# udaysankar01/xfeatSLAM

Hardware: AMD Instinct MI355X
Metric: XFeat frames/s (VGA, 4096 kpts) + 4096x4096 desc-match pairs/s (higher is better)
Workload: dtype f32

## Files before the change

### xfeatslam_amd/csrc/kernels_conv.hip

```cpp
#include "ctx.h"
#include "heads_kp4.hip.h"
#include <stdlib.h>

struct ConvArgs {
    const float* in;
    StatSrc st;
    size_t in_stride;
    int Hin, Win;
    const float* w;
    const float* bias;
    float* out;
    size_t out_stride;
    int Hout, Wout;
    double* part;
    size_t part_stride;
    int tiles_x;
    const float* pool; size_t pool_stride; const float* skip_w; const float* skip_b;
    const float* r4; size_t s4; int H4, W4; StatSrc st4;
    const float* r5; size_t s5; int H5, W5; StatSrc st5;
    const float* xstat; const float* w0; const float* bias0;
    int dbg;
};

enum { PRO_PLAIN = 0, PRO_BN = 1, PRO_IN = 2, PRO_B2IN = 3, PRO_FUSE = 4, PRO_L0 = 5, PRO_UNFOLD = 6, PRO_FUSEA = 7  };
enum { EPI_STATS = 0, EPI_BIAS = 1, EPI_BIAS_RELU = 2 };

#ifdef XFH_STAMPS
__device__ unsigned long long g_stamps[32 * 8];
#define XFH_STAMP(a, ph) do { if (blockIdx.x == gridDim.x / 2 && blockIdx.y == 0 && blockIdx.z == 0 && threadIdx.x == 0) g_stamps[((a).dbg & 31) * 8 + (ph)] = wall_clock64(); } while (0)
extern "C" int xfh_debug_stamps(unsigned long long* out) { return (int)hipMemcpyFromSymbol(out, HIP_SYMBOL(g_stamps), sizeof g_stamps); }
#define XFH_STAMP_ROW(row, ph) do { if (blockIdx.x == gridDim.x / 2 && blockIdx.y == 0 && blockIdx.z == 0 && threadIdx.x == 0) g_stamps[(row) * 8 + (ph)] = wall_clock64(); } while (0)
#else
#define XFH_STAMP(a, ph) do { } while (0)
#define XFH_STAMP_ROW(row, ph) do { } while (0)
#endif

__device__ __forceinline__ void lin_coeff_c(int in, int out, int d, int& i0, int& i1, float& l0, float& l1) {
    const float scale = (float)in / (float)out;
    float src = fmaf(scale, (float)d + 0.5f, -0.5f);
    if (src < 0.f) src = 0.f;
    int a = (int)src;
    if (a > in - 1) a = in - 1;
    float lam = src - (float)a;
    lam = fminf(fmaxf(lam, 0.f), 1.f);
    i0 = a; i1 = a + ((a < in - 1) ? 1 : 0);
    l1 = lam; l0 = 1.f - lam;
}
template <bool ACT = false>
__device__ __forceinline__ void ld_act8(const float* __restrict__ raw, const float* st, size_t pix, int g, f32x4& v0, f32x4& v1) {
    const float* p = raw + pix * 64 + g * 8;
    v0 = *(const f32x4*)p; v1 = *(const f32x4*)(p + 4);
    if constexpr (ACT) return;
#pragma unroll
    for (int q = 0; q < 4; ++q) {
        v0[q] = fmaxf(fmaf(v0[q], st[64 + g * 8 + q], st[g * 8 + q]), 0.f);
        v1[q] = fmaxf(fmaf(v1[q], st[64 + g * 8 + 4 + q], st[g * 8 + 4 + q]), 0.f);
    }
}
template <bool ACT = false>
__device__ __forceinline__ void up_bilinear8(const float* __restrict__ raw, const float* st, int Hi, int Wi, int Ho, int Wo, int y, int x, int g, f32x4& o0, f32x4& o1) {
    int y0, y1, x0, x1; float hy0, hy1, wx0, wx1;
    lin_coeff_c(Hi, Ho, y, y0, y1, hy0, hy1);
    lin_coeff_c(Wi, Wo, x, x0, x1, wx0, wx1);
    f32x4 a0, a1, b0, b1, c0, c1, d0, d1;
    ld_act8<ACT>(raw, st, (size_t)y0 * Wi + x0, g, a0, a1); ld_act8<ACT>(raw, st, (size_t)y0 * Wi + x1, g, b0, b1);
    ld_act8<ACT>(raw, st, (size_t)y1 * Wi + x0, g, c0, c1); ld_act8<ACT>(raw, st, (size_t)y1 * Wi + x1, g, d0, d1);
#pragma unroll
    for (int j = 0; j < 4; ++j) {
        const float t0 = fmaf(wx0, a0[j], wx1 * b0[j]), u0 = fmaf(wx0, c0[j], wx1 * d0[j]);
        o0[j] = fmaf(hy0, t0, hy1 * u0);
        const float t1 = fmaf(wx0, a1[j], wx1 * b1[j]), u1 = fmaf(wx0, c1[j], wx1 * d1[j]);
        o1[j] = fmaf(hy0, t1, hy1 * u1);
    }
}

__global__ __launch_bounds__(256)
void k_act_pyramid(const float* __restrict__ raw4, size_t s4, const float* __restrict__ st4, int n4 ,
                   const float* __restrict__ raw5, size_t s5, const float* __restrict__ st5, int n5, float* __restrict__ act4, float* __restrict__ act5) {
    const int b = blockIdx.z;
    for (int q = blockIdx.x * 256 + threadIdx.x; q < (n4 + n5) / 4; q += gridDim.x * 256) {
        const bool five = q >= n4 / 4;
        const int e = (five ? q - n4 / 4 : q) * 4, ch = e & 63;
        const float* st = (five ? st5 : st4) + (size_t)b * 128;
        const size_t off = (size_t)b * (five ? s5 : s4) + e;
        f32x4 v = *(const f32x4*)((five ? raw5 : raw4) + off);
        const f32x4 be = *(const f32x4*)(st + ch), al = *(const f32x4*)(st + 64 + ch);
#pragma unroll
        for (int j = 0; j < 4; ++j) v[j] = fmaxf(fmaf(v[j], al[j], be[j]), 0.f);
        *(f32x4*)((five ? act5 : act4) + off) = v;
    }
}

__global__ __launch_bounds__(256)
void k_bn_finalize(const double* __restrict__ part, size_t part_stride, int npart, int C, double count,
                   float* __restrict__ stat ) {
    __shared__ double red[256 * 2];
    const int b = blockIdx.x;
    bn_fold<16>(part + (size_t)b * part_stride, npart, C, count, stat + (size_t)b * 2 * C, red, threadIdx.x, 256);
}

__device__ __forceinline__ double wave_sum_f64(double v) {
    v += __shfl_xor(v, 32); v += __shfl_xor(v, 16); v += __shfl_xor(v, 8);
    v += __shfl_xor(v, 4); v += __shfl_xor(v, 2); v += __shfl_xor(v, 1);
    return v;
}
typedef float f32x2 __attribute__((ext_vector_type(2)));
__device__ __forceinline__ void l0_conv(const float (&win)[9], const XFH_CONST float* __restrict__ w, float (&acc)[4]) {
    f32x2 a0 = {0.f, 0.f}, a1 = {0.f, 0.f};
#pragma unroll
    for (int k = 0; k < 9; ++k) {
        const f32x2 v = {win[k], win[k]};
        a0 = __builtin_elementwise_fma(v, f32x2{w[k * 4], w[k * 4 + 1]}, a0);
        a1 = __builtin_elementwise_fma(v, f32x2{w[k * 4 + 2], w[k * 4 + 3]}, a1);
    }
    acc[0] = a0.x; acc[1] = a0.y; acc[2] = a1.x; acc[3] = a1.y;
}

constexpr int L0S_TW = 128, L0S_TH = 32, L0S_R = 4;
__global__ __launch_bounds__(256)
void k_block1_stats(const float* __restrict__ X, size_t x_stride, StatSrc xs, int H, int W, int tiles_x,
                    const float* __restrict__ w0, double* __restrict__ part, size_t part_stride, float* __restrict__ pool, size_t pool_stride) {
    __shared__ double s_red[512];
    __shared__ float s_xst[2];
    const int t = threadIdx.x, b = blockIdx.z, tile = blockIdx.x;
    XFH_STAMP_ROW(0, 0);
    const int gx = (tile % tiles_x) * L0S_TW + (t & 31) * 4, gy0 = (tile / tiles_x) * L0S_TH + (t >> 5) * L0S_R;
    const float* x = X + (size_t)b * x_stride;
    f32x4 rv[L0S_R + 2]; float rl[L0S_R + 2], rr[L0S_R + 2];
    {
        const int cx = min(gx, W - 4), cl = max(min(gx, W) - 1, 0), cr = min(gx + 4, W - 1);
#pragma unroll
        for (int i = 0; i < L0S_R + 2; ++i) {
            const float* p = x + (size_t)min(max(gy0 - 1 + i, 0), H - 1) * W;
            rv[i] = *(const f32x4*)(p + cx); rl[i] = p[cl]; rr[i] = p[cr];
        }
    }
    XFH_STAMP_ROW(0, 1);
    stage_stat<16>(xs, b, 1, tile == 0, s_xst, s_red, t, 256);
    XFH_STAMP_ROW(0, 2);
    const float m = s_xst[0], r = s_xst[1];
    auto load_row = [&](int i, float (&row)[6]) {
        const int gy = gy0 - 1 + i;
        const bool iny = gy >= 0 && gy < H;
        const f32x4 v = rv[i];
        const bool inx = iny && gx < W;
        row[1] = inx ? fmaf(v.x, r, m) : 0.f; row[2] = inx ? fmaf(v.y, r, m) : 0.f; row[3] = inx ? fmaf(v.z, r, m) : 0.f; row[4] = inx ? fmaf(v.w, r, m) : 0.f;
        row[0] = (iny && gx > 0 && gx - 1 < W) ? fmaf(rl[i], r, m) : 0.f;
        row[5] = (iny && gx + 4 < W) ? fmaf(rr[i], r, m) : 0.f;
    };
    float win[3][6];
    load_row(0, win[0]);
    load_row(1, win[1]);
    double sum[4] = {0.0, 0.0, 0.0, 0.0}, sq[4] = {0.0, 0.0, 0.0, 0.0};
    float ps = 0.f;
#pragma unroll
    for (int i = 0; i < L0S_R; ++i) {
        load_row(i + 2, win[(i + 2) % 3]);
        const float (&r0)[6] = win[i % 3], (&r1)[6] = win[(i + 1) % 3], (&r2)[6] = win[(i + 2) % 3];
#pragma unroll
        for (int q = 0; q < 4; ++q) ps += r1[q + 1];
#pragma unroll
        for (int q = 0; q < 4; ++q) {
            const float wq[9] = {r0[q], r0[q + 1], r0[q + 2], r1[q], r1[q + 1], r1[q + 2], r2[q], r2[q + 1], r2[q + 2]};
            float acc[4];
            l0_conv(wq, (const XFH_CONST float*)w0, acc);
            if (gy0 + i < H && gx + q < W) {
#pragma unroll
                for (int co = 0; co < 4; ++co) { const double d = (double)acc[co]; sum[co] += d; sq[co] = fma(d, d, sq[co]); }
            }
        }
    }
    XFH_STAMP_ROW(0, 4);
#pragma unroll
    for (int co = 0; co < 4; ++co) { sum[co] = wave_sum_f64(sum[co]); sq[co] = wave_sum_f64(sq[co]); }
    if (gy0 < H && gx < W) pool[(size_t)b * pool_stride + (size_t)(gy0 >> 2) * (W >> 2) + (gx >> 2)] = ps / 16.0f;
    if ((t & 63) == 0) {
#pragma unroll
        for (int co = 0; co < 4; ++co) { s_red[(t >> 6) * 8 + co * 2] = sum[co]; s_red[(t >> 6) * 8 + co * 2 + 1] = sq[co]; }
    }
    __syncthreads();
    if (t < 8)
        part[(size_t)b * part_stride + (size_t)tile * 8 + t] = (s_red[t] + s_red[8 + t]) + (s_red[16 + t] + s_red[24 + t]);
    XFH_STAMP_ROW(0, 5);
}

__device__ __forceinline__ int xcd_tile(int x, int n) {
    const int k = x & 7, q = n >> 3, r = n & 7;
    return k * q + (k < r ? k : r) + (x >> 3);
}

template <int CIN, int COUT, int ST, int PRO, bool FOLD, int EPI>
__global__ __launch_bounds__(256)
void k_conv_direct(ConvArgs a) {
    constexpr int TI = 15 * ST + 3;
    constexpr int SL = 256 / COUT;
    static_assert(PRO != PRO_L0 || (CIN == 4 && ST == 2 && COUT == 8), "PRO_L0 is block1.1");
    constexpr int XW = TI + 2, XS = XW + 1;
    constexpr int SIN = TI * TI * CIN > 256 * (COUT + 1) ? TI * TI * CIN : 256 * (COUT + 1);
    __shared__ __attribute__((aligned(16))) float s_in[SIN];
    float* s_out = s_in;
    __shared__ __attribute__((aligned(16))) float s_xwin[PRO == PRO_L0 ? XW * XS : 1];
    __shared__ double s_red[FOLD ? 512 : 8 * COUT];
    constexpr bool WLDS = FOLD;
    constexpr int NWQ = 9 * CIN * COUT / 4;
    __shared__ __attribute__((aligned(16))) float s_wt[WLDS ? NWQ * 4 : 4];
    const int t = threadIdx.x, b = blockIdx.z;
    XFH_STAMP(a, 0);
    const int tile = xcd_tile(blockIdx.x, gridDim.x), tx0 = (tile % a.tiles_x) * 16, ty0 = (tile / a.tiles_x) * 16;
    const float* in = a.in + (size_t)b * a.in_stride;
    __shared__ float s_stat[FOLD ? 2 * CIN : 1];
    static_assert(NWQ <= 256, "one weight quad per thread");
    f32x4 wq4 = {0.f, 0.f, 0.f, 0.f};
    if (WLDS && t < NWQ) wq4 = *(const f32x4*)(a.w + t * 4);
    const float* st = a.st.stat + (size_t)b * 2 * (PRO == PRO_IN ? 1 : CIN);

    constexpr int VEC = (CIN >= 4) ? 4 : 1;
    constexpr int G = CIN / VEC;
    if constexpr (PRO == PRO_L0) {
        float* s_x = s_xwin;
        const float xm = a.xstat[b * 2], xr = a.xstat[b * 2 + 1];
        constexpr int NX = (XW * XW + 255) / 256;
        float xv[NX];
#pragma unroll
        for (int k = 0; k < NX; ++k) {
            const int item = t + k * 256, iy = item / XW, ix = item % XW;
            const int gy = ty0 * ST - 2 + iy, gx = tx0 * ST - 2 + ix;
            xv[k] = in[(size_t)min(max(gy, 0), a.Hin - 1) * a.Win + min(max(gx, 0), a.Win - 1)];
        }
        if constexpr (FOLD) stage_stat<16>(a.st, b, CIN, tile == 0, s_stat, s_red, t, 256);
#pragma unroll
        for (int k = 0; k < NX; ++k) {
            const int item = t + k * 256, iy = item / XW, ix = item % XW;
            const int gy = ty0 * ST - 2 + iy, gx = tx0 * ST - 2 + ix;
            const bool ok = gy >= 0 && gy < a.Hin && gx >= 0 && gx < a.Win;
            if (item < XW * XW) s_x[iy * XS + ix] = ok ? fmaf(xv[k], xr, xm) : 0.f;
        }
        __syncthreads();
        for (int pix = t; pix < TI * TI; pix += 256) {
            const int iy = pix / TI, ix = pix % TI;
            const int gy = ty0 * ST - 1 + iy, gx = tx0 * ST - 1 + ix;
            f32x4 v = {0.f, 0.f, 0.f, 0.f};
            if (gy >= 0 && gy < a.Hin && gx >= 0 && gx < a.Win) {
                const float* sp = s_x + iy * XS + ix;
                const float win[9] = {sp[0], sp[1], sp[2], sp[XS], sp[XS + 1], sp[XS + 2], sp[2 * XS], sp[2 * XS + 1], sp[2 * XS + 2]};
                float acc[4];
                l0_conv(win, (const XFH_CONST float*)a.w0, acc);
#pragma unroll
                for (int q = 0; q < 4; ++q) {
                    if constexpr (EPI == EPI_BIAS_RELU) v[q] = fmaxf(acc[q] + a.bias0[q], 0.f);
                    else {
                        const float m = FOLD ? s_stat[q] : st[q], r = FOLD ? s_stat[CIN + q] : st[CIN + q];
                        v[q] = fmaxf(fmaf(acc[q], r, m), 0.f);
                    }
                }
            }
            *(f32x4*)(s_in + pix * CIN) = v;
        }
    } else
    {
        constexpr int NI = (TI * TI + 255) / 256;
        f32x4 iv[NI][G];
#pragma unroll
        for (int k = 0; k < NI; ++k) {
            const int pix = t + k * 256;
            const int gy = min(max(ty0 * ST - 1 + pix / TI, 0), a.Hin - 1), gx = min(max(tx0 * ST - 1 + pix % TI, 0), a.Win - 1);
            const float* p = in + ((size_t)gy * a.Win + gx) * CIN;
#pragma unroll
            for (int g = 0; g < G; ++g) {
                if constexpr (VEC == 4) iv[k][g] = *(const f32x4*)(p + g * 4);
                else iv[k][g].x = p[0];
            }
        }
        if constexpr (FOLD) stage_stat<16>(a.st, b, CIN, tile == 0, s_stat, s_red, t, 256);
#pragma unroll
        for (int k = 0; k < NI; ++k) {
            const int pix = t + k * 256;
            const int gy = ty0 * ST - 1 + pix / TI, gx = tx0 * ST - 1 + pix % TI;
            const bool ok = gy >= 0 && gy < a.Hin && gx >= 0 && gx < a.Win;
            if (pix >= TI * TI) continue;
            if constexpr (VEC == 4) {
#pragma unroll
                for (int g = 0; g < G; ++g) {
                    f32x4 v = iv[k][g];
#pragma unroll
                    for (int q = 0; q < 4; ++q) {
                        const float m = FOLD ? s_stat[g * 4 + q] : st[g * 4 + q], r = FOLD ? s_stat[CIN + g * 4 + q] : st[CIN + g * 4 + q];
                        v[q] = ok ? fmaxf(fmaf(v[q], r, m), 0.f) : 0.f;
                    }
                    *(f32x4*)(s_in + pix * CIN + g * 4) = v;
                }
            } else {
                s_in[pix] = ok ? fmaf(iv[k][0].x, st[1], st[0]) : 0.f;
            }
        }
    }
    if (WLDS && t < NWQ) *(f32x4*)(s_wt + t * 4) = wq4;
    __syncthreads();
    XFH_STAMP(a, 3);

    const int tx = t & 15, ty = t >> 4;
    float acc[COUT];
#pragma unroll
    for (int co = 0; co < COUT; ++co) acc[co] = 0.f;
#pragma unroll
    for (int ky = 0; ky < 3; ++ky)
#pragma unroll
        for (int kx = 0; kx < 3; ++kx) {
            const float* sp = s_in + ((ty * ST + ky) * TI + tx * ST + kx) * CIN;
            float v[CIN];
            if constexpr (VEC == 4) {
#pragma unroll
                for (int g = 0; g < G; ++g) {
                    const f32x4 q = *(const f32x4*)(sp + g * 4);
                    v[g * 4 + 0] = q.x; v[g * 4 + 1] = q.y; v[g * 4 + 2] = q.z; v[g * 4 + 3] = q.w;
                }
            } else {
                v[0] = sp[0];
            }
#pragma unroll
            for (int ci = 0; ci < CIN; ++ci) {
                if constexpr (WLDS) {
                    const float* wr = s_wt + ((ky * 3 + kx) * CIN + ci) * COUT;
#pragma unroll
                    for (int g4 = 0; g4 < COUT / 4; ++g4) {
                        const f32x4 w4 = *(const f32x4*)(wr + g4 * 4);
#pragma unroll
                        for (int e = 0; e < 4; ++e) acc[g4 * 4 + e] = fmaf(v[ci], w4[e], acc[g4 * 4 + e]);
                    }
                } else {
                    const float* wr = a.w + ((ky * 3 + kx) * CIN + ci) * COUT;
#pragma unroll
                    for (int co = 0; co < COUT; ++co) acc[co] = fmaf(v[ci], wr[co], acc[co]);
                }
            }
        }

    XFH_STAMP(a, 4);
    const int oy = ty0 + ty, ox = tx0 + tx;
    const bool valid = oy < a.Hout && ox < a.Wout;
    if constexpr (EPI == EPI_BIAS_RELU) {
#pragma unroll
        for (int co = 0; co < COUT; ++co) acc[co] = fmaxf(acc[co] + a.bias[co], 0.f);
    }
    if (valid) {
        float* o = a.out + (size_t)b * a.out_stride + ((size_t)oy * a.Wout + ox) * COUT;
#pragma unroll
        for (int g = 0; g < COUT / 4; ++g)
            *(f32x4*)(o + g * 4) = f32x4{acc[g * 4], acc[g * 4 + 1], acc[g * 4 + 2], acc[g * 4 + 3]};
    }
    if constexpr (EPI != EPI_STATS) return;
    __syncthreads();
#pragma unroll
    for (int co = 0; co < COUT; ++co) s_out[t * (COUT + 1) + co] = valid ? acc[co] : 0.f;
    __syncthreads();
    {
        const int c = t % COUT, j = t / COUT;
        double s = 0.0, ss = 0.0;
#pragma unroll
        for (int p = 0; p < 256 / SL; ++p) {
            const double v = (double)s_out[(j + p * SL) * (COUT + 1) + c];
            s += v; ss = fma(v, v, ss);
        }
#pragma unroll
        for (int off = COUT; off < 64; off <<= 1) { s += __shfl_xor(s, off); ss += __shfl_xor(ss, off); }
        if ((t & 63) < COUT) { s_red[((t >> 6) * COUT + c) * 2] = s; s_red[((t >> 6) * COUT + c) * 2 + 1] = ss; }
    }
    __syncthreads();
    if (t < 2 * COUT)
        a.part[(size_t)b * a.part_stride + (size_t)tile * COUT * 2 + t] = (s_red[t] + s_red[2 * COUT + t]) + (s_red[4 * COUT + t] + s_red[6 * COUT + t]);
    XFH_STAMP(a, 5);
}

typedef unsigned u32x4_t __attribute__((ext_vector_type(4)));
__device__ __forceinline__ __amdgpu_buffer_rsrc_t wbuf_make(const float* w) { return __builtin_amdgcn_make_buffer_rsrc((void*)w, 0, 0x7fffffff, 0x00020000); }
__device__ __forceinline__ f32x4 wbuf_ld(__amdgpu_buffer_rsrc_t r, int f , int chunk_float_off ) {
    return __builtin_bit_cast(f32x4, __builtin_amdgcn_raw_buffer_load_b128(r, (unsigned)f * 16u, chunk_float_off * 4, 0));
}
template <int COUT, int NT, int EPI>
__device__ __forceinline__ void conv_bias(const float* __restrict__ bias, int co0, float (&bv)[NT]) {
#pragma unroll
    for (int n = 0; n < NT; ++n) {
        bv[n] = 0.f;
        if constexpr (EPI != EPI_STATS) bv[n] = (COUT % 32 == 0 || co0 + n * 32 < COUT) ? bias[co0 + n * 32] : 0.f;
    }
}

template <int COUT, int NT, int WW, int WH, int EPI>
__device__ __forceinline__ void conv_epilogue(const f32x16 (&acc)[NT], float* __restrict__ wave_out , int Wout,
                                              int rows_left, int cols_left, int co0, int h, const float (&bias)[NT] ,
                                              double (&sum)[NT], double (&sq)[NT]) {
    static_assert(WW >= 8 && WW * WH == 32, "pixel block of a wave");
    XFH_MFMA_SETTLE();
    const bool full = rows_left >= WH && cols_left >= WW;
    const int lane_off = 4 * h * COUT + co0;
    const int rowstride = Wout * COUT;
    auto value = [&](int n, int r, float* dst, float bv) {
        float v = acc[n][r];
        if constexpr (EPI != EPI_STATS) v += bv;
        if constexpr (EPI == EPI_BIAS_RELU) v = fmaxf(v, 0.f);
        dst[lane_off] = v;
        if constexpr (EPI == EPI_STATS) { const double dv = (double)v; sum[n] += dv; sq[n] = fma(dv, dv, sq[n]); }
    };
    if (full) {
#pragma unroll
        for (int n = 0; n < NT; ++n) {
            sum[n] = 0.0; sq[n] = 0.0;
            if (COUT % 32 == 0 || co0 + n * 32 < COUT) {
#pragma unroll
                for (int r = 0; r < 16; ++r) {
                    const int pb = (r & 3) + 8 * (r >> 2);
                    value(n, r, wave_out + (pb / WW) * rowstride + (pb % WW) * COUT + n * 32, bias[n]);
                }
            }
        }
        return;
    }
#pragma unroll
    for (int n = 0; n < NT; ++n) {
        const int co = co0 + n * 32;
        sum[n] = 0.0; sq[n] = 0.0;
        const float bv = bias[n];
        const bool cok = COUT % 32 == 0 || co < COUT;
#pragma unroll
        for (int r = 0; r < 16; ++r) {
            const int pb = (r & 3) + 8 * (r >> 2);
            const int prow = pb / WW, pcol = pb % WW;
            float* dst = wave_out + prow * rowstride + pcol * COUT + n * 32;
            if (cok && prow < rows_left && pcol + 4 * h < cols_left) value(n, r, dst, bv);
        }
    }
}

#ifndef XFH_PD
#define XFH_PD 3
#endif

template <int CIN, int COUT, int KS, int ST, int WM, int WN, int NT, int WW, int PRO, int EPI, int CBMAX = 64, int TPC = 1, int PD = XFH_PD>
__device__ __forceinline__ void conv_mfma_body(const ConvArgs a, const int tile, const int b, float* smem) {
    constexpr int NTHR = 64 * WM * WN;
    constexpr int WH = 32 / WW, TH = WM * WH, TW = WW;
    constexpr int COUTP = WN * NT * 32;
    constexpr int PAD = KS / 2;
    constexpr int TIH = (TH - 1) * ST + KS, TIW = (TW - 1) * ST + KS;
    constexpr int CP = CIN + 4;
    constexpr int CB = CIN > CBMAX ? CBMAX : CIN;
    constexpr int NCB = CIN / CB;
    static_assert(TPC == 1 || NCB == 1, "several taps per chunk only with all channels in the chunk");
    static_assert((KS * KS) % TPC == 0, "taps per chunk");
    constexpr int NCHUNK = KS * KS * NCB / TPC;
    constexpr int NWBUF = NCHUNK > 1 ? 2 : 1;
    constexpr int KC = TPC * CB;
    constexpr int WS = KC + 4;
    constexpr int WCH = COUTP * KC;
    constexpr int NWLD = (WCH / 4 + NTHR - 1) / NTHR;
    constexpr int G = CIN / 8;
    constexpr int IN_FLOATS = TIH * TIW * CP;
    constexpr int W_FLOATS = COUTP * WS;

    float* s_in = smem;
    float* s_w = smem + IN_FLOATS;
    float* s_stat = s_w + NWBUF * W_FLOATS;

    const int t = threadIdx.x;
    const int tx0 = (tile % a.tiles_x) * TW, ty0 = (tile / a.tiles_x) * TH;
    const float* in = a.in + (size_t)b * a.in_stride;

    XFH_STAMP(a, 0);
    f32x4 wreg[PD][NWLD];
    const __amdgpu_buffer_rsrc_t wrs = wbuf_make(a.w);
#pragma unroll
    for (int c = 0; c < PD; ++c)
#pragma unroll
        for (int q = 0; q < NWLD; ++q) {
            const int f = t + q * NTHR;
            if (c < NCHUNK && f < WCH / 4) wreg[c][q] = wbuf_ld(wrs, f, c * WCH);
        }
    constexpr int NITEM = TIH * TIW * G;
    constexpr int NIT = (NITEM + NTHR - 1) / NTHR;
    constexpr bool FUSE = PRO == PRO_FUSE || PRO == PRO_FUSEA;
    constexpr bool BATCHED = !FUSE;
    f32x4 r0[BATCHED ? NIT : 1], r1[BATCHED ? NIT : 1];
    float rp[PRO == PRO_B2IN ? NIT : 1];
    if constexpr (BATCHED) {
#pragma unroll
        for (int k = 0; k < NIT; ++k) {
            const int item = t + k * NTHR, pix = item / G, g = item % G;
            const int gy = min(max(ty0 * ST - PAD + pix / TIW, 0), a.Hin - 1), gx = min(max(tx0 * ST - PAD + pix % TIW, 0), a.Win - 1);
            const float* p = PRO == PRO_UNFOLD ? in + ((size_t)(gy * 8 + g) * (a.Win * 8) + gx * 8) : in + ((size_t)gy * a.Win + gx) * CIN + g * 8;
            r0[k] = *(const f32x4*)p;
            r1[k] = *(const f32x4*)(p + 4);
            if constexpr (PRO == PRO_B2IN) rp[k] = a.pool[(size_t)b * a.pool_stride + (size_t)gy * a.Win + gx];
        }
    }
    XFH_STAMP(a, 1);
    if constexpr (PRO == PRO_BN || PRO == PRO_B2IN || FUSE) stage_stat(a.st, b, CIN, tile == 0, s_stat, (double*)s_in, t, NTHR);
    if constexpr (PRO == PRO_B2IN) {
        for (int q = t; q < CIN; q += NTHR) { s_stat[2 * CIN + q] = a.skip_w[q]; s_stat[3 * CIN + q] = a.skip_b[q]; }
        __syncthreads();
    }
    if constexpr (PRO == PRO_FUSE) {
        stage_stat(a.st4, b, 64, tile == 0, s_stat + 128, (double*)s_in, t, NTHR);
        stage_stat(a.st5, b, 64, tile == 0, s_stat + 256, (double*)s_in, t, NTHR);
    }
    XFH_STAMP(a, 2);
    if constexpr (BATCHED) {
#pragma unroll
        for (int k = 0; k < NIT; ++k) {
            const int item = t + k * NTHR, pix = item / G, g = item % G;
            const int gy = ty0 * ST - PAD + pix / TIW, gx = tx0 * ST - PAD + pix % TIW;
            const bool ok = gy >= 0 && gy < a.Hin && gx >= 0 && gx < a.Win;
            if (NITEM % NTHR != 0 && item >= NITEM) continue;
            f32x4 v0 = r0[k], v1 = r1[k];
            if constexpr (PRO == PRO_UNFOLD) {
                const float xm = a.xstat[b * 2], xr = a.xstat[b * 2 + 1];
#pragma unroll
                for (int q = 0; q < 4; ++q) { v0[q] = fmaf(v0[q], xr, xm); v1[q] = fmaf(v1[q], xr, xm); }
            }
            if constexpr (PRO == PRO_BN || PRO == PRO_B2IN) {
                const f32x4 m0 = *(const f32x4*)(s_stat + g * 8), m1 = *(const f32x4*)(s_stat + g * 8 + 4);
                const f32x4 q0 = *(const f32x4*)(s_stat + CIN + g * 8), q1 = *(const f32x4*)(s_stat + CIN + g * 8 + 4);
#pragma unroll
                for (int q = 0; q < 4; ++q) {
                    v0[q] = fmaxf(fmaf(v0[q], q0[q], m0[q]), 0.f);
                    v1[q] = fmaxf(fmaf(v1[q], q1[q], m1[q]), 0.f);
                }
            }
            if constexpr (PRO == PRO_B2IN) {
                const float pl = rp[k];
#pragma unroll
                for (int q = 0; q < 4; ++q) {
                    v0[q] = v0[q] + (pl * s_stat[2 * CIN + g * 8 + q] + s_stat[3 * CIN + g * 8 + q]);
                    v1[q] = v1[q] + (pl * s_stat[2 * CIN + g * 8 + 4 + q] + s_stat[3 * CIN + g * 8 + 4 + q]);
                }
            }
            if constexpr (KS > 1) { if (!ok) { v0 = f32x4{0.f, 0.f, 0.f, 0.f}; v1 = v0; } }
            float* d = s_in + pix * CP + g * 8;
            *(f32x4*)d = f32x4{v0.x, v0.z, v1.x, v1.z};
            *(f32x4*)(d + 4) = f32x4{v0.y, v0.w, v1.y, v1.w};
        }
    } else
    for (int item = t; item < TIH * TIW * G; item += NTHR) {
        const int pix = item / G, g = item % G;
        const int iy = pix / TIW, ix = pix % TIW;
        const int gy = ty0 * ST - PAD + iy, gx = tx0 * ST - PAD + ix;
        f32x4 v0 = {0.f, 0.f, 0.f, 0.f}, v1 = {0.f, 0.f, 0.f, 0.f};
        if (gy >= 0 && gy < a.Hin && gx >= 0 && gx < a.Win) {
            const float* p = in + ((size_t)gy * a.Win + gx) * CIN + g * 8;
            v0 = *(const f32x4*)p;
            v1 = *(const f32x4*)(p + 4);
#pragma unroll
            for (int q = 0; q < 4; ++q) {
                v0[q] = fmaxf(fmaf(v0[q], s_stat[CIN + g * 8 + q], s_stat[g * 8 + q]), 0.f);
                v1[q] = fmaxf(fmaf(v1[q], s_stat[CIN + g * 8 + 4 + q], s_stat[g * 8 + 4 + q]), 0.f);
            }
            f32x4 u0, u1, w0, w1;
            up_bilinear8<PRO == PRO_FUSEA>(a.r4 + (size_t)b * a.s4, s_stat + 128, a.H4, a.W4, a.Hin, a.Win, gy, gx, g, u0, u1);
            up_bilinear8<PRO == PRO_FUSEA>(a.r5 + (size_t)b * a.s5, s_stat + 256, a.H5, a.W5, a.Hin, a.Win, gy, gx, g, w0, w1);
#pragma unroll
            for (int q = 0; q < 4; ++q) { v0[q] = (v0[q] + u0[q]) + w0[q]; v1[q] = (v1[q] + u1[q]) + w1[q]; }
        }
        float* d = s_in + pix * CP + g * 8;
        *(f32x4*)d = f32x4{v0.x, v0.z, v1.x, v1.z};
        *(f32x4*)(d + 4) = f32x4{v0.y, v0.w, v1.y, v1.w};
    }
#pragma unroll
    for (int q = 0; q < NWLD; ++q) {
        const int f = t + q * NTHR;
        if (f < WCH / 4) {
            const int n = f / (KC / 4), c4 = f % (KC / 4);
            *(f32x4*)(s_w + n * WS + c4 * 4) = wreg[0][q];
            if (PD < NCHUNK) wreg[0][q] = wbuf_ld(wrs, f, PD * WCH);
        }
    }
    __syncthreads();
    XFH_STAMP(a, 3);

    const int wave = __builtin_amdgcn_readfirstlane(t >> 6), lane = t & 63, i = lane & 31, h = lane >> 5;
    const int wm = wave / WN, wn = wave % WN;
    const int pr = i / WW, pc = i % WW;
    const int ly = (wm * WH + pr) * ST, lx = pc * ST;

    float biasv[NT];
    conv_bias<COUT, NT, EPI>(a.bias, wn * NT * 32 + i, biasv);
    f32x16 acc[NT];
#pragma unroll
    for (int n = 0; n < NT; ++n)
#pragma unroll
        for (int r = 0; r < 16; ++r) acc[n][r] = 0.f;

#pragma unroll
    for (int ch = 0; ch < NCHUNK; ++ch) {
#pragma unroll
        for (int tt = 0; tt < TPC; ++tt) {
            const int tap = TPC == 1 ? ch / NCB : ch * TPC + tt, cb = TPC == 1 ? ch % NCB : 0;
            const int ky = tap / KS, kx = tap % KS;
            const float* pa = s_in + ((ly + ky) * TIW + lx + kx) * CP + cb * CB + 4 * h;
            const float* pw = s_w + (ch & 1) * W_FLOATS + (wn * NT * 32 + i) * WS + tt * CB + 4 * h;
#pragma unroll
            for (int kk = 0; kk < CB / 8; ++kk) {
                const f32x4 av = *(const f32x4*)(pa + kk * 8);
#pragma unroll
                for (int n = 0; n < NT; ++n) {
                    const f32x4 bv = *(const f32x4*)(pw + n * 32 * WS + kk * 8);
#pragma unroll
                    for (int j = 0; j < 4; ++j)
                        acc[n] = __builtin_amdgcn_mfma_f32_32x32x2f32(av[j], bv[j], acc[n], 0, 0, 0);
                }
            }
        }
        if (ch + 1 < NCHUNK) {
            float* wd = s_w + ((ch + 1) & 1) * W_FLOATS;
#pragma unroll
            for (int q = 0; q < NWLD; ++q) {
                const int f = t + q * NTHR;
                if (f < WCH / 4) {
                    const int n = f / (KC / 4), c4 = f % (KC / 4);
                    *(f32x4*)(wd + n * WS + c4 * 4) = wreg[(ch + 1) % PD][q];
                    if (ch + 1 + PD < NCHUNK) wreg[(ch + 1) % PD][q] = wbuf_ld(wrs, f, (ch + 1 + PD) * WCH);
                }
            }
        }
        __syncthreads();
    }

    XFH_STAMP(a, 4);
    double sum[NT], sq[NT];
    {
        const int oy0 = ty0 + wm * WH;
        float* wave_out = a.out + (size_t)b * a.out_stride + ((size_t)oy0 * a.Wout + tx0) * COUT;
        conv_epilogue<COUT, NT, WW, WH, EPI>(acc, wave_out, a.Wout, a.Hout - oy0, a.Wout - tx0, wn * NT * 32 + i, h, biasv, sum, sq);
    }
    if constexpr (EPI == EPI_STATS) {
        double* s_red = (double*)smem;
// ... 1220 lines not shown
```

Baseline: 32340.

## Restructure block1 prologue staging with interior fast path and row-strip L0 conv

Rewrites the input-staging prologue of the fused block1 conv kernel. The L0 path now loads the input window as float pairs, skips clamping and bounds masks for interior tiles, and has each thread compute a vertical strip of 5 output rows while reusing a sliding 3-row register window instead of reloading 9 LDS values per pixel. The BN path is specialised to exactly 2 vector groups with a fixed load split and the same interior/border specialisation. Weight and stat pointers are cast to the constant address space so they can use scalar loads. This adds template specialisation and static_asserts that tie the code to the block1 shapes, and relies on in-bounds pair loads at the right edge.

```diff
diff --git a/xfeatslam_amd/csrc/kernels_conv.hip b/xfeatslam_amd/csrc/kernels_conv.hip
--- a/xfeatslam_amd/csrc/kernels_conv.hip
+++ b/xfeatslam_amd/csrc/kernels_conv.hip
@@ -1,6 +1,7 @@
 #include "ctx.h"
 #include "heads_kp4.hip.h"
 #include <stdlib.h>
+#include <type_traits>
 
 struct ConvArgs {
     const float* in;
@@ -212,87 +213,115 @@
     static_assert(NWQ <= 256, "one weight quad per thread");
     f32x4 wq4 = {0.f, 0.f, 0.f, 0.f};
     if (WLDS && t < NWQ) wq4 = *(const f32x4*)(a.w + t * 4);
-    const float* st = a.st.stat + (size_t)b * 2 * (PRO == PRO_IN ? 1 : CIN);
+    const XFH_CONST float* st = (const XFH_CONST float*)a.st.stat + (size_t)b * 2 * (PRO == PRO_IN ? 1 : CIN);
 
     constexpr int VEC = (CIN >= 4) ? 4 : 1;
     constexpr int G = CIN / VEC;
     if constexpr (PRO == PRO_L0) {
         float* s_x = s_xwin;
         const float xm = a.xstat[b * 2], xr = a.xstat[b * 2 + 1];
-        constexpr int NX = (XW * XW + 255) / 256;
-        float xv[NX];
-#pragma unroll
-        for (int k = 0; k < NX; ++k) {
-            const int item = t + k * 256, iy = item / XW, ix = item % XW;
-            const int gy = ty0 * ST - 2 + iy, gx = tx0 * ST - 2 + ix;
-            xv[k] = in[(size_t)min(max(gy, 0), a.Hin - 1) * a.Win + min(max(gx, 0), a.Win - 1)];
-        }
-        if constexpr (FOLD) stage_stat<16>(a.st, b, CIN, tile == 0, s_stat, s_red, t, 256);
-#pragma unroll
-        for (int k = 0; k < NX; ++k) {
-            const int item = t + k * 256, iy = item / XW, ix = item % XW;
-            const int gy = ty0 * ST - 2 + iy, gx = tx0 * ST - 2 + ix;
-            const bool ok = gy >= 0 && gy < a.Hin && gx >= 0 && gx < a.Win;
-            if (item < XW * XW) s_x[iy * XS + ix] = ok ? fmaf(xv[k], xr, xm) : 0.f;
-        }
-        __syncthreads();
-        for (int pix = t; pix < TI * TI; pix += 256) {
-            const int iy = pix / TI, ix = pix % TI;
-            const int gy = ty0 * ST - 1 + iy, gx = tx0 * ST - 1 + ix;
-            f32x4 v = {0.f, 0.f, 0.f, 0.f};
-            if (gy >= 0 && gy < a.Hin && gx >= 0 && gx < a.Win) {
-                const float* sp = s_x + iy * XS + ix;
-                const float win[9] = {sp[0], sp[1], sp[2], sp[XS], sp[XS + 1], sp[XS + 2], sp[2 * XS], sp[2 * XS + 1], sp[2 * XS + 2]};
-                float acc[4];
-                l0_conv(win, (const XFH_CONST float*)a.w0, acc);
+        constexpr int NP = XS / 2, NX = (XW * NP + 255) / 256;
+        static_assert(XS == 2 * NP && XW <= XS, "a row of s_x is a whole number of pairs");
+        const int wy0 = ty0 * ST - 2, wx0 = tx0 * ST - 2;
+        const bool inner = wy0 >= 0 && wy0 + XW <= a.Hin && wx0 >= 0 && wx0 + XS <= a.Win;
+        auto stage = [&](auto inner_c) {
+            constexpr bool IN = decltype(inner_c)::value;
+            float sm[4], sr[4];
+            auto load_st = [&]() {
 #pragma unroll
                 for (int q = 0; q < 4; ++q) {
-                    if constexpr (EPI == EPI_BIAS_RELU) v[q] = fmaxf(acc[q] + a.bias0[q], 0.f);
-                    else {
-                        const float m = FOLD ? s_stat[q] : st[q], r = FOLD ? s_stat[CIN + q] : st[CIN + q];
-                        v[q] = fmaxf(fmaf(acc[q], r, m), 0.f);
+                    if constexpr (EPI == EPI_BIAS_RELU) { sm[q] = a.bias0[q]; sr[q] = 0.f; }
+                    else { sm[q] = FOLD ? s_stat[q] : st[q]; sr[q] = FOLD ? s_stat[CIN + q] : st[CIN + q]; }
+                }
+            };
+            if constexpr (!FOLD) load_st();
+            f32x2 xv[NX];
+#pragma unroll
+            for (int k = 0; k < NX; ++k) {
+                const int item = min(t + k * 256, XW * NP - 1);
+                int gy = wy0 + item / NP, gx = wx0 + (item % NP) * 2;
+                if constexpr (!IN) { gy = min(max(gy, 0), a.Hin - 1); gx = min(max(gx, 0), a.Win - 2); }
+                xv[k] = *(const f32x2*)(in + (size_t)gy * a.Win + gx);
+            }
+            asm volatile("" ::: "memory");
+            if constexpr (FOLD) { stage_stat<16>(a.st, b, CIN, tile == 0, s_stat, s_red, t, 256); load_st(); }
+#pragma unroll
+            for (int k = 0; k < NX; ++k) {
+                const int item = t + k * 256;
+                f32x2 v = {fmaf(xv[k].x, xr, xm), fmaf(xv[k].y, xr, xm)};
+                if constexpr (!IN) {
+                    const int gy = wy0 + item / NP, gx = wx0 + (item % NP) * 2;
+                    const bool ok = gy >= 0 && gy < a.Hin && gx >= 0 && gx < a.Win;
+                    v.x = ok ? v.x : 0.f; v.y = ok ? v.y : 0.f;
+                }
+                if ((k + 1) * 256 <= XW * NP || item < XW * NP) *(f32x2*)(s_x + item * 2) = v;
+            }
+            __syncthreads();
+            constexpr int RC = 5, NS = (TI + RC - 1) / RC, RL = TI - (NS - 1) * RC;
+            static_assert(NS * TI <= 256 && NS * RC <= XW && RL + 2 <= RC, "one strip per thread; no read below s_x, and the last strip's stored rows need no clamped row");
+            if (t < NS * TI) {
+                const int strip = t / TI, ix = t % TI, iy0 = strip * RC;
+                const float* sp = s_x + iy0 * XS + ix;
+                const float* sq = s_x + min(iy0 + RC, XW - 2) * XS + ix;
+                float rw[RC + 2][3];
+#pragma unroll
+                for (int i = 0; i < RC + 2; ++i)
+#pragma unroll
+                    for (int j = 0; j < 3; ++j) rw[i][j] = i < RC ? sp[i * XS + j] : sq[(i - RC) * XS + j];
+#pragma unroll
+                for (int i = 0; i < RC; ++i) {
+                    const float win[9] = {rw[i][0], rw[i][1], rw[i][2], rw[i + 1][0], rw[i + 1][1], rw[i + 1][2], rw[i + 2][0], rw[i + 2][1], rw[i + 2][2]};
+                    float acc[4];
+                    l0_conv(win, (const XFH_CONST float*)a.w0, acc);
+                    f32x4 v;
+#pragma unroll
+                    for (int q = 0; q < 4; ++q) {
+                        if constexpr (EPI == EPI_BIAS_RELU) v[q] = fmaxf(acc[q] + sm[q], 0.f);
+                        else v[q] = fmaxf(fmaf(acc[q], sr[q], sm[q]), 0.f);
                     }
-                }
-            }
-            *(f32x4*)(s_in + pix * CIN) = v;
-        }
+                    if constexpr (!IN) {
+                        const int gy = ty0 * ST - 1 + iy0 + i, gx = tx0 * ST - 1 + ix;
+                        if (!(gy >= 0 && gy < a.Hin && gx >= 0 && gx < a.Win)) v = f32x4{0.f, 0.f, 0.f, 0.f};
+                    }
+                    if (i < RL || strip < NS - 1) *(f32x4*)(s_in + ((iy0 + i) * TI + ix) * CIN) = v;
+                }
+            }
+        };
+        if (inner) stage(std::true_type{}); else stage(std::false_type{});
     } else
     {
-        constexpr int NI = (TI * TI + 255) / 256;
-        f32x4 iv[NI][G];
-#pragma unroll
-        for (int k = 0; k < NI; ++k) {
-            const int pix = t + k * 256;
-            const int gy = min(max(ty0 * ST - 1 + pix / TI, 0), a.Hin - 1), gx = min(max(tx0 * ST - 1 + pix % TI, 0), a.Win - 1);
-            const float* p = in + ((size_t)gy * a.Win + gx) * CIN;
-#pragma unroll
-            for (int g = 0; g < G; ++g) {
-                if constexpr (VEC == 4) iv[k][g] = *(const f32x4*)(p + g * 4);
-                else iv[k][g].x = p[0];
-            }
-        }
-        if constexpr (FOLD) stage_stat<16>(a.st, b, CIN, tile == 0, s_stat, s_red, t, 256);
-#pragma unroll
-        for (int k = 0; k < NI; ++k) {
-            const int pix = t + k * 256;
-            const int gy = ty0 * ST - 1 + pix / TI, gx = tx0 * ST - 1 + pix % TI;
-            const bool ok = gy >= 0 && gy < a.Hin && gx >= 0 && gx < a.Win;
-            if (pix >= TI * TI) continue;
-            if constexpr (VEC == 4) {
-#pragma unroll
-                for (int g = 0; g < G; ++g) {
-                    f32x4 v = iv[k][g];
-#pragma unroll
-                    for (int q = 0; q < 4; ++q) {
-                        const float m = FOLD ? s_stat[g * 4 + q] : st[g * 4 + q], r = FOLD ? s_stat[CIN + g * 4 + q] : st[CIN + g * 4 + q];
-                        v[q] = ok ? fmaxf(fmaf(v[q], r, m), 0.f) : 0.f;
-                    }
-                    *(f32x4*)(s_in + pix * CIN + g * 4) = v;
-                }
-            } else {
-                s_in[pix] = ok ? fmaf(iv[k][0].x, st[1], st[0]) : 0.f;
-            }
-        }
+        static_assert(PRO == PRO_BN && G == 2 && TI * TI > 256 && TI * TI - 256 <= 128, "block1.2");
+        constexpr int NT = TI * TI - 256;
+        const int wy0 = ty0 * ST - 1, wx0 = tx0 * ST - 1;
+        const bool inner = wy0 >= 0 && wy0 + TI <= a.Hin && wx0 >= 0 && wx0 + TI <= a.Win;
+        const int g2 = __builtin_amdgcn_readfirstlane(t >> 7), pix2 = 256 + min(t & 127, NT - 1);
+        auto stage = [&](auto inner_c) {
+            constexpr bool IN = decltype(inner_c)::value;
+            auto src = [&](int pix) {
+                int gy = wy0 + pix / TI, gx = wx0 + pix % TI;
+                if constexpr (!IN) { gy = min(max(gy, 0), a.Hin - 1); gx = min(max(gx, 0), a.Win - 1); }
+                return in + ((size_t)gy * a.Win + gx) * CIN;
+            };
+            const float* p = src(t);
+            f32x4 iv[3] = {*(const f32x4*)p, *(const f32x4*)(p + 4), *(const f32x4*)(src(pix2) + g2 * 4)};
+            asm volatile("" ::: "memory");
+            if constexpr (FOLD) stage_stat<16>(a.st, b, CIN, tile == 0, s_stat, s_red, t, 256);
+            auto put = [&](f32x4 v, int pix, int g) {
+                bool ok = true;
+                if constexpr (!IN) { const int gy = wy0 + pix / TI, gx = wx0 + pix % TI; ok = gy >= 0 && gy < a.Hin && gx >= 0 && gx < a.Win; }
+#pragma unroll
+                for (int q = 0; q < 4; ++q) {
+                    const float m = FOLD ? s_stat[g * 4 + q] : st[g * 4 + q], r = FOLD ? s_stat[CIN + g * 4 + q] : st[CIN + g * 4 + q];
+                    v[q] = fmaxf(fmaf(v[q], r, m), 0.f);
+                    if constexpr (!IN) v[q] = ok ? v[q] : 0.f;
+                }
+                *(f32x4*)(s_in + pix * CIN + g * 4) = v;
+            };
+            put(iv[0], t, 0);
+            put(iv[1], t, 1);
+            if ((t & 127) < NT) { if (g2 == 0) put(iv[2], pix2, 0); else put(iv[2], pix2, 1); }
+        };
+        if (inner) stage(std::true_type{}); else stage(std::false_type{});
     }
     if (WLDS && t < NWQ) *(f32x4*)(s_wt + t * 4) = wq4;
     __syncthreads();
@@ -328,7 +357,7 @@
                         for (int e = 0; e < 4; ++e) acc[g4 * 4 + e] = fmaf(v[ci], w4[e], acc[g4 * 4 + e]);
                     }
                 } else {
-                    const float* wr = a.w + ((ky * 3 + kx) * CIN + ci) * COUT;
+                    const XFH_CONST float* wr = (const XFH_CONST float*)a.w + ((ky * 3 + kx) * CIN + ci) * COUT;
 #pragma unroll
                     for (int co = 0; co < COUT; ++co) acc[co] = fmaf(v[ci], wr[co], acc[co]);
                 }
```

Measured after the change: 32530, median of 5. Within noise of the previous version (+0.6%).
